# YifanXu74/MQ-Det

Hardware: AMD Instinct MI355X
Metric: images/sec MQ-GLIP-T 800×1333 5-shot vision queries, 1/2/4/8 MI355X (higher is better)
Workload: dtype f16; 1 GPU; BASELINE.json configs[1]: MQ-GLIP-T (Swin-T + BERT-base + GCP + 6-layer VLDyHead), 5 vision queries x 40 classes, 141-token caption, LVIS-style post-processing; every step a full forward (feature / language caches OFF; only host-side tokenizer / query-selection results are memoised)); global_batch=8, batch_per_gpu=8, image=800x1333 -> 800x1344, parallelism=dp1, weights=seeded random init (no checkpoints offline), residual_streams=fp32

## Files before the change

include/mqdet_hip.h:

```cpp
#ifndef MQDET_HIP_H
#define MQDET_HIP_H
#ifdef __cplusplus
extern "C" {
#endif

int mq_abi_version(void);

long mq_attn_workspace_bytes(int B, int H, int Nq, int D, int nsplit);
int mq_attn_fwd(const void* q, const void* k, const void* vt, void* o, const float* key_bias, const int* kv_len,
                const unsigned char* qk_mask, long mask_bs, long mask_hs, long mask_rs, void* workspace,
                int B, int H, int Nq, int Nk, int D,
                long q_bs, long q_rs, long q_hs, long k_bs, long k_rs, long k_hs, long vt_bs, long vt_rs, long vt_hs,
                long o_bs, long o_rs, long bias_bs, long bias_hs, float scale, float clamp, int nsplit, void* stream);

int mq_attn_resident_fwd(const void* q, const void* k, const void* vt, void* o, const float* key_bias, const int* kv_len,
                         const unsigned char* qk_mask, long mask_bs, long mask_hs, long mask_rs, int B, int H, int Nq, int Nk, int D,
                         long q_bs, long q_rs, long q_hs, long k_bs, long k_rs, long k_hs, long vt_bs, long vt_rs, long vt_hs,
                         long o_bs, long o_rs, long bias_bs, long bias_hs, float scale, float clamp, void* stream);

int mq_attn_chunked_fwd(const void* q, const void* k, const void* vt, void* o, const float* key_bias, const int* kv_len,
                        void* workspace, int B, int H, int Nq, int Nk, int D,
                        long q_bs, long q_rs, long q_hs, long k_bs, long k_rs, long k_hs, long vt_bs, long vt_rs, long vt_hs,
                        long o_bs, long o_rs, long bias_bs, long bias_hs, float scale, float clamp, int nsplit, void* stream);

// ... 80 lines not shown
int mq_add_upsample_nearest(void* dst, const void* src, int B, int H, int W, int Hc, int Wc, int C, void* stream);
int mq_dyrelu_ln_fwd(const void* x, long x_bs, const float* coef, const int* row_first, int NL, const void* gamma, const void* beta,
                     float eps, void* y, int B, int N, int C, void* stream);

int mq_align_scores_fwd(const void* dot, int dot_f32, const float* tbias, const int* tokidx, long tok_bs, const void* ctr,
                        float* out, float* cls_out, int B, int HW, int T, int L, int MT, float thr, long dot_bs, int agg,
                        void* stream);

int mq_align_fused_fwd(const void* tok, const void* tk, const float* tbias, const void* wbc, const float* bbc, const float* scales,
                       const int* tokidx, long tok_bs, const int* lvl_off, float* ranked, float* cls_out, float* reg, float* ctr_out,
                       float* logits, int B, int N, int T, int kv_max, int L, int MT, int NL, float thr, int agg, void* stream);

int mq_box_decode(const float* val, const long* flat, const void* reg, int reg_f32, const float* anchors, const int* label_ids, long lab_bs,
                  const float* im_wh, float* boxes, float* scores, int* labels, int B, int K, int HW, int L,
                  long out_stride, long out_off, void* stream);

int mq_roi_align_fwd(const void* feat, int feat_f32, const float* rois, float* out, int R, int C, int H, int W,
                     long sn, long sc, long sh, long sw, int PH, int PW, float spatial_scale, int sampling_ratio,
                     int aligned, int reduce_mean, void* stream);

int mq_msdeform_attn_fwd(const void* value, int value_f32, const long* shapes, const long* level_start, const float* loc,
                         const float* attn, void* out, int out_f32, int B, int S, int M, int D, int L, int Q, int P, void* stream);

int mq_msdeform_attn_q_fwd(const void* value, int value_f32, long value_bs, long value_ts, const long* shapes,
                           const long* level_start, const void* qproj, const float* ref, int ref_dim, const int* valid_hw,
                           void* out, int out_f32, int B, int S, int M, int D, int L, int Q, int P, void* stream);

long mq_ml_nms_workspace_bytes(int B, int N);
int mq_ml_nms(const float* boxes, const int* labels, const int* nvalid, void* workspace, unsigned char* keep,
              int B, int N, float thr, void* stream);

int mq_ml_nms_topk(const float* boxes, const int* labels, const int* nvalid, void* workspace, unsigned char* keep,
                   int B, int N, float thr, int max_keep, void* stream);

int mq_patch_embed_fwd(const void* img, int img_f32, const void* w, const float* bias, const float* g0, const float* b0, const float* g1,
                       const float* b1, float* x32, void* h1, int B, int Hi, int Wi, int C, float eps, void* stream);

int mq_attn_text_fwd(const void* q, const void* k, const void* v, void* o, const float* key_bias, const int* kv_len,
                     int B, int H, int Nq, int Nk, int D, long q_bs, long q_rs, long q_hs, long k_bs, long k_rs, long k_hs,
                     long v_bs, long v_rs, long v_hs, long o_bs, long o_rs, long bias_bs, long bias_hs, float scale,
                     float clamp, int max_kv, void* stream);

long mq_post_select_workspace_bytes(const int* hw, const int* k, int NL, int B, int L);
int mq_post_select_fwd(const float* const* ranked, const float* const* reg, const float* const* anchors, const int* hw, const int* k,
                       int NL, int B, int L, const int* label_ids, long lab_bs, const float* im_wh, void* workspace, float* boxes,
                       float* scores, int* labels, int* ids, void* stream);
int mq_post_sort_fwd(const float* boxes, const float* scores, const int* labels, const int* off, int NL, float* boxes_o, float* scores_o,
                     int* labels_o, int* nvalid, int B, int tot, void* stream);
int mq_post_finalize_fwd(const float* boxes, const float* scores, const int* labels, const unsigned char* keep, float* out,
                         int* counts, int B, int tot, int K, int K2, void* stream);

int mq_tta_ingest_fwd(const unsigned char* src, const long* src_off, const int* meta, const int* bounds, const int* coef, float* out,
                      float* out_flip, int* err, int B, int Hp, int Wp, int TH, int R, const float* mean, const float* stdv, int bgr, int x255,
                      void* stream);
int mq_tta_merge_prep(const float* packed, const int* counts, const float* tparam, const float* band, const int* cls_rank,
                      int n_cls, float* boxes, float* scores, int* labels, unsigned char* valid, float* boxes_s, float* scores_s,
                      int* labels_s, int* src_s, int* nvalid, int* ndrop, int T, int B, int K, void* stream);
int mq_tta_merge_finalize(const float* boxes_s, const float* scores_s, const int* labels_s, const int* src_s, const unsigned char* keep,
                          const int* nvalid, float* thr, const int* cls_rank, float* boxes_o, float* scores_o, long long* labels_o, int* counts, int B, int N,
                          int top_n, void* stream);
int mq_tta_merge_special(const float* boxes_s, const float* scores_s, const int* labels_s, const int* src_s, const int* nvalid,
                         const int* cls_rank, float* boxes_m, float* scores_m, unsigned char* keep, int* seq, float* ws, int* nws, int B,
                         int N, int L, int mode, float thresh, float aux, int cap, void* stream);
int mq_tta_merge_finalize_special(const float* boxes_m, const float* scores_m, const int* labels_s, const int* seq,
                                  const unsigned char* keep, const int* nvalid, float* thr, const int* cls_rank, float* boxes_o,
                                  float* scores_o, long long* labels_o, int* counts, int B, int N, int top_n, void* stream);
// ... 130 lines not shown
```

mq_det_amd/build.py:

```python
import os
import subprocess
import sys

HERE = os.path.dirname(os.path.abspath(__file__))
CSRC = os.path.join(HERE, "csrc")
LIB_DIR = os.path.join(HERE, "lib")
LIB = os.path.join(LIB_DIR, "libmqdet_hip.so")
SOURCES = ["api.hip", "attn.hip", "attn_resident.hip", "attn_text.hip", "bert_attn.hip", "vlfuse_attn.hip", "window_attn.hip", "patch_embed.hip", "gcp.hip", "gcp_fused.hip", "conv_igemm.hip", "conv_small.hip", "conv_small2.hip", "conv_small3.hip", "dcn_fused.hip", "layernorm.hip", "layernorm2.hip", "dyconv.hip", "post.hip", "post2.hip", "align_fused.hip", "nms2.hip", "roi_align.hip", "swin_mlp2.hip", "msda.hip", "tta.hip", "lvis_eval.hip", "coco_eval.hip", "flickr_eval.hip", "query_bank.hip"]
F32_SKIP = ("roi_align.hip", "nms2.hip", "post2.hip", "tta.hip", "lvis_eval.hip", "coco_eval.hip", "flickr_eval.hip", "query_bank.hip")
FLAGS = ["--offload-arch=gfx950", "-O3", "-std=c++17", "-fPIC"]
EXTRA_FLAGS = {"dcn_fused.hip": ["-fno-slp-vectorize"],
               "swin_mlp2.hip": ["-fno-slp-vectorize"],
               "attn_resident.hip": ["-fno-slp-vectorize", "-mllvm", "-amdgpu-mfma-vgpr-form"],
               "attn_text.hip": ["-fno-slp-vectorize", "-mllvm", "-amdgpu-mfma-vgpr-form"],
               "bert_attn.hip": ["-fno-slp-vectorize", "-mllvm", "-amdgpu-mfma-vgpr-form"]}


STAMP = os.path.join(LIB_DIR, "libmqdet_hip.stamp")


def _digest():
    import hashlib
    h = hashlib.sha256()
    deps = sorted(os.path.join(CSRC, f) for f in os.listdir(CSRC)) + [os.path.join(HERE, "..", "include", "mqdet_hip.h"), os.path.abspath(__file__)]
    for d in deps:
        if os.path.isfile(d):
            with open(d, "rb") as f:
                h.update(os.path.basename(d).encode() + b"\0" + f.read())
    return h.hexdigest()


def _stale():
    if not os.path.exists(LIB) or not os.path.exists(STAMP):
        return True
    with open(STAMP) as f:
        return f.read().strip() != _digest()


def build(force=False, verbose=True):
    if not force and not _stale():
        return LIB
    os.makedirs(LIB_DIR, exist_ok=True)
# ... 29 lines not shown
```

mq_det_amd/csrc/nms2.hip:

```cpp
#include "common.h"

MQ_NAMESPACE_BEGIN
#ifdef MQ_PRIMARY_UNIT

__device__ __forceinline__ float ml_iou2(const float* a, int la, const float* b, int lb) {
  if (la != lb) return 0.f;
  float left = fmaxf(a[0], b[0]), right = fminf(a[2], b[2]);
  float top = fmaxf(a[1], b[1]), bottom = fminf(a[3], b[3]);
  float w = fmaxf(right - left + 1.f, 0.f), h = fmaxf(bottom - top + 1.f, 0.f);
  float inter = w * h;
  float sa = (a[2] - a[0] + 1.f) * (a[3] - a[1] + 1.f);
  float sb = (b[2] - b[0] + 1.f) * (b[3] - b[1] + 1.f);
  return inter / (sa + sb - inter);
}

__global__ __launch_bounds__(64) void nms2_mask_kernel(const float* __restrict__ boxes, const int* __restrict__ labels,
                                                      const int* __restrict__ nvalid, unsigned long long* __restrict__ mask,
                                                      int N, int col_blocks, float thr) {
  const int b = blockIdx.z, row_blk = blockIdx.y, col_blk = blockIdx.x;
  const int n = nvalid[b];
  if (row_blk * 64 >= n || col_blk * 64 >= n || col_blk < row_blk) {
    int i = row_blk * 64 + threadIdx.x;
    if (i < N) mask[((long)b * N + i) * col_blocks + col_blk] = 0ULL;
    return;
  }
  __shared__ float cb[64 * 4];
  __shared__ int cl[64];
  const float* bb = boxes + (long)b * N * 4;
  const int* lb = labels + (long)b * N;
  const int cj = col_blk * 64 + threadIdx.x;
  if (cj < n) {
    cb[threadIdx.x * 4 + 0] = bb[cj * 4 + 0]; cb[threadIdx.x * 4 + 1] = bb[cj * 4 + 1];
    cb[threadIdx.x * 4 + 2] = bb[cj * 4 + 2]; cb[threadIdx.x * 4 + 3] = bb[cj * 4 + 3];
    cl[threadIdx.x] = lb[cj];
  }
  __syncthreads();
  const int i = row_blk * 64 + threadIdx.x;
  unsigned long long t = 0ULL;
  if (i < n) {
    float a[4] = {bb[i * 4 + 0], bb[i * 4 + 1], bb[i * 4 + 2], bb[i * 4 + 3]};
    int la = lb[i];
    int cols = min(64, n - col_blk * 64);
    int start = (row_blk == col_blk) ? threadIdx.x + 1 : 0;
    for (int j = start; j < cols; ++j)
      if (ml_iou2(a, la, cb + j * 4, cl[j]) > thr) t |= 1ULL << j;
  }
  if (i < N) mask[((long)b * N + i) * col_blocks + col_blk] = t;
// ... 116 lines not shown
```

mq_det_amd/ops.py:

```python
import ctypes
import math
import os

import torch

_LIB = None
_LIB_PATH = os.path.join(os.path.dirname(os.path.abspath(__file__)), "lib", "libmqdet_hip.so")

_vp, _i, _l, _f = ctypes.c_void_p, ctypes.c_int, ctypes.c_long, ctypes.c_float
EXPECTED_ABI = 31
_SIGNATURES = {
    "mq_abi_version": (_i, []),
    "mq_attn_workspace_bytes": (_l, [_i, _i, _i, _i, _i]),
    "mq_attn_fwd": (_i, [_vp, _vp, _vp, _vp, _vp, _vp, _vp, _l, _l, _l, _vp, _i, _i, _i, _i, _i] + [_l] * 13 + [_f, _f, _i, _vp]),
    "mq_attn_resident_fwd": (_i, [_vp, _vp, _vp, _vp, _vp, _vp, _vp, _l, _l, _l, _i, _i, _i, _i, _i] + [_l] * 13 + [_f, _f, _vp]),
    "mq_patch_embed_fwd": (_i, [_vp, _i, _vp, _vp, _vp, _vp, _vp, _vp, _vp, _vp, _i, _i, _i, _i, _f, _vp]),
    "mq_attn_text_fwd": (_i, [_vp, _vp, _vp, _vp, _vp, _vp, _i, _i, _i, _i, _i] + [_l] * 13 + [_f, _f, _i, _vp]),
    "mq_bert_attn_qkv_fwd": (_i, [_vp, _vp, _vp, _vp, _vp, _vp, _i, _i, _i, _i, _l, _l, _l, _l, _l, _f, _f, _vp]),
    "mq_attn_chunked_fwd": (_i, [_vp, _vp, _vp, _vp, _vp, _vp, _vp, _i, _i, _i, _i, _i] + [_l] * 13 + [_f, _f, _i, _vp]),
    "mq_window_attn_fwd": (_i, [_vp, _vp, _vp, _vp, _i, _i, _i, _i, _i, _i, _i, _vp]),
    "mq_window_attn_qkv_fwd": (_i, [_vp, _vp, _vp, _vp, _vp, _i, _i, _i, _i, _i, _i, _i, _vp]),
    "mq_gcp_sparse_attn_fwd": (_i, [_vp, _vp, _vp, _vp, _i, _i, _i, _i, _i, _i, _vp]),
    "mq_gcp_gate_residual_fwd": (_i, [_vp, _vp, _vp, _vp, _i, _vp, _vp, _l, _i, _i, _vp]),
    "mq_gcp_attn_fwd": (_i, [_vp] * 16 + [_l, _i, _i, _i, _i, _i, _i, _i, _f, _i, _vp]),
# ... 6 lines not shown
    "mq_clamp_gelu_clamp": (_i, [_vp, _vp, _l, _f, _vp]),
    "mq_patch_merge_ln_fwd": (_i, [_vp, _i, _vp, _vp, _vp, _i, _i, _i, _i, _f, _vp]),
    "mq_swin_mlp2_fwd": (_i, [_vp, _vp, _vp, _vp, _f, _vp, _vp, _vp, _vp, _vp, _vp, _vp, _f, _vp, _l, _i, _i, _vp]),
    "mq_conv3x3_fwd": (_i, [_vp, _vp, _vp, _vp, _i, _i, _i, _i, _l, _i, _i, _i, _vp]),
    "mq_conv3x3_nchw32_fwd": (_i, [_vp, _vp, _vp, _vp, _i, _i, _i, _i, _l, _i, _vp]),
    "mq_conv3x3_nchw32_v2_fwd": (_i, [_vp, _vp, _vp, _vp, _i, _i, _i, _i, _l, _i, _vp]),
    "mq_conv3x3_nchw32_group_fwd": (_i, [_vp, _i, _vp, _vp, _i, _i, _i, _vp]),
    "mq_dcnv2_stats_blocks": (_i, [_i, _i, _i]),
    "mq_dcnv2_fwd": (_i, [_vp, _vp, _vp, _vp, _vp, _vp, _vp, _vp, _i, _i, _i, _i, _l, _i, _i, _i, _i, _i, _i, _vp]),
    "mq_dcnv2_group_fwd": (_i, [_vp, _i, _vp]),
    "mq_dyconv_stats": (_i, [_vp, _vp, _vp, _vp, _i, _i, _i, _i, _vp]),
    "mq_dyconv_coef": (_i, [_vp, _vp, _vp, _vp, _vp, _vp, _i, _i, _i, _i, _i, _f, _i, _vp]),
    "mq_dyconv_coef_group": (_i, [_vp, _i, _vp, _vp, _i, _i, _i, _f, _vp]),
    "mq_dyconv_fuse": (_i, [_vp, _vp, _i, _i, _vp, _vp, _i, _i, _vp, _vp, _i, _i, _i, _vp, _l, _vp, _i, _i, _i, _i, _vp]),
    "mq_dyrelu_coef": (_i, [_vp, _vp, _vp, _vp, _vp, _vp, _i, _i, _i, _vp]),
    "mq_dyconv_epilogue_group": (_i, [_vp, _i, _vp, _vp, _vp, _vp, _i, _i, _vp]),
    "mq_add_upsample_nearest": (_i, [_vp, _vp, _i, _i, _i, _i, _i, _i, _vp]),
    "mq_pool2x2_tokens_fwd": (_i, [_vp, _i, _vp, _i, _i, _vp]),
    "mq_dyrelu_ln_fwd": (_i, [_vp, _l, _vp, _vp, _i, _vp, _vp, _f, _vp, _i, _i, _i, _vp]),
    "mq_dyrelu_apply": (_i, [_vp, _vp, _i, _i, _i, _l, _vp]),
    "mq_align_scores_fwd": (_i, [_vp, _i, _vp, _vp, _l, _vp, _vp, _vp, _i, _i, _i, _i, _i, _f, _l, _i, _vp]),
    "mq_align_fused_fwd": (_i, [_vp, _vp, _vp, _vp, _vp, _vp, _vp, _l, _vp, _vp, _vp, _vp, _vp, _vp, _i, _i, _i, _i, _i, _i, _i, _f, _i, _vp]),
    "mq_box_decode": (_i, [_vp, _vp, _vp, _i, _vp, _vp, _l, _vp, _vp, _vp, _vp, _i, _i, _i, _i, _l, _l, _vp]),
    "mq_roi_align_fwd": (_i, [_vp, _i, _vp, _vp, _i, _i, _i, _i, _l, _l, _l, _l, _i, _i, _f, _i, _i, _i, _vp]),
    "mq_msdeform_attn_fwd": (_i, [_vp, _i, _vp, _vp, _vp, _vp, _vp, _i, _i, _i, _i, _i, _i, _i, _i, _vp]),
    "mq_msdeform_attn_q_fwd": (_i, [_vp, _i, _l, _l, _vp, _vp, _vp, _vp, _i, _vp, _vp, _i, _i, _i, _i, _i, _i, _i, _i, _vp]),
    "mq_post_select_workspace_bytes": (_l, [_vp, _vp, _i, _i, _i]),
    "mq_post_select_fwd": (_i, [_vp, _vp, _vp, _vp, _vp, _i, _i, _i, _vp, _l, _vp, _vp, _vp, _vp, _vp, _vp, _vp]),
    "mq_post_sort_fwd": (_i, [_vp, _vp, _vp, _vp, _i, _vp, _vp, _vp, _vp, _i, _i, _vp]),
    "mq_post_finalize_fwd": (_i, [_vp, _vp, _vp, _vp, _vp, _vp, _i, _i, _i, _i, _vp]),
    "mq_ml_nms_workspace_bytes": (_l, [_i, _i]),
    "mq_ml_nms_topk": (_i, [_vp, _vp, _vp, _vp, _vp, _i, _i, _f, _i, _vp]),
    "mq_ml_nms": (_i, [_vp, _vp, _vp, _vp, _vp, _i, _i, _f, _vp]),
    "mq_tta_ingest_fwd": (_i, [_vp] * 8 + [_i] * 5 + [_vp, _vp, _i, _i, _vp]),
    "mq_tta_merge_prep": (_i, [_vp] * 5 + [_i] + [_vp] * 10 + [_i, _i, _i, _vp]),
    "mq_tta_merge_finalize": (_i, [_vp] * 12 + [_i, _i, _i, _vp]),
    "mq_tta_merge_special": (_i, [_vp] * 12 + [_i, _i, _i, _i, _f, _f, _i, _vp]),
    "mq_tta_merge_finalize_special": (_i, [_vp] * 12 + [_i, _i, _i, _vp]),
    "mq_tta_merge_nms": (_i, [_vp] * 7 + [_i, _i, _i, _f, _i, _vp]),
    "mq_lvis_match": (_i, [_vp] * 13 + [_i, _l, _vp]),
    "mq_lvis_accumulate": (_i, [_vp] * 7 + [_i, _vp]),
    "mq_coco_match": (_i, [_vp] * 12 + [_i, _l, _vp]),
    "mq_coco_accumulate": (_i, [_vp] * 9 + [_i, _vp]),
    "mq_flickr_recall": (_i, [_vp] * 7 + [_i, _i, _vp]),
    "mq_flickr_tally": (_i, [_vp] * 5 + [_i, _i, _i, _vp]),
    "mq_bank_admit": (_i, [_vp] * 8 + [_i] * 8 + [_f, _vp]),
}
BF16_TWINS = ("mq_attn_fwd", "mq_attn_resident_fwd", "mq_attn_text_fwd", "mq_bert_attn_qkv_fwd", "mq_patch_embed_fwd", "mq_attn_chunked_fwd", "mq_window_attn_fwd", "mq_window_attn_qkv_fwd", "mq_gcp_sparse_attn_fwd", "mq_gcp_gate_residual_fwd", "mq_gcp_attn_fwd", "mq_vlfuse_i2t_fwd", "mq_vlfuse_t2i_fwd",
              "mq_layernorm_fwd", "mq_layernorm2_fwd", "mq_layernorm_clamp_fwd", "mq_clamp_gelu_clamp", "mq_patch_merge_ln_fwd", "mq_swin_mlp2_fwd", "mq_conv3x3_fwd", "mq_conv3x3_nchw32_fwd", "mq_conv3x3_nchw32_v2_fwd", "mq_conv3x3_nchw32_group_fwd", "mq_dcnv2_fwd", "mq_dcnv2_group_fwd",
              "mq_dyconv_stats", "mq_dyconv_coef", "mq_dyconv_coef_group", "mq_dyconv_fuse", "mq_dyrelu_coef", "mq_dyconv_epilogue_group", "mq_dyrelu_apply", "mq_dyrelu_ln_fwd", "mq_add_upsample_nearest", "mq_pool2x2_tokens_fwd",
              "mq_align_scores_fwd", "mq_align_fused_fwd", "mq_box_decode", "mq_roi_align_fwd", "mq_msdeform_attn_fwd", "mq_msdeform_attn_q_fwd")
F32_TWINS = tuple(n for n in BF16_TWINS if n not in ("mq_roi_align_fwd",))
for _n in BF16_TWINS:
    _SIGNATURES[_n + "_bf16"] = _SIGNATURES[_n]
for _n in F32_TWINS:
    _SIGNATURES[_n + "_f32"] = _SIGNATURES[_n]
EXPORTS = tuple(_SIGNATURES)


from .selection import KERNEL_DEFAULTS, KERNELS, _ThreadLocalTable, configure, activate


def lib_path():
    return _LIB_PATH


# ... 1196 lines not shown

def ms_deform_attn_q(value, spatial_shapes, qproj, ref, heads, out_dtype=None, valid_hw=None):
    lib = load_library()
    _need_gpu(value, qproj, ref)
    B, S, C = value.shape
    D = C // heads
    Q = qproj.shape[1]
    shapes = tuple((int(h), int(w)) for h, w in spatial_shapes)
    L, P = len(shapes), 4
    assert sum(h * w for h, w in shapes) == S and value.stride(2) == 1 and value.dtype in _H16 + (torch.float32,)
    assert qproj.dtype in _H16 and qproj.is_contiguous() and qproj.shape == (B, Q, heads * L * P * 3)
    assert ref.dtype == torch.float32 and ref.is_contiguous() and ref.shape[:3] == (B, Q, L) and ref.shape[3] in (2, 4)
    if valid_hw is not None:
        _need_gpu(valid_hw)
        assert valid_hw.dtype == torch.int32 and valid_hw.is_contiguous() and valid_hw.shape == (B, L, 2)
    hw, start = _msda_shapes(shapes, value.device)
    out_dtype = out_dtype or value.dtype
    out = torch.empty(B, Q, C, dtype=out_dtype, device=value.device)
    nb = B * S * C * value.element_size() + qproj.numel() * 2 + ref.numel() * 4 + out.numel() * out.element_size()
    with _timed(f"msdeform_attn_q{Q}", nb):
        _chk(_fn(lib, "mq_msdeform_attn_q_fwd", value, qproj, out)(_ptr(value), int(value.dtype == torch.float32), value.stride(0), value.stride(1), _ptr(hw),
                                        _ptr(start), _ptr(qproj), _ptr(ref), ref.shape[3], _ptr(valid_hw), _ptr(out),
                                        int(out_dtype == torch.float32), B, S, heads, D, L, Q, P, _stream()),
             "mq_msdeform_attn_q_fwd")
    return out


def ml_nms(boxes, labels, nvalid, thresh, max_keep=0, as_bool=True):
    lib = load_library()
    _need_gpu(boxes, labels, nvalid)
    B, N, _ = boxes.shape
    assert boxes.is_contiguous() and labels.is_contiguous() and boxes.dtype == torch.float32
    assert labels.dtype == torch.int32 and nvalid.dtype == torch.int32
    ws = torch.empty(max(lib.mq_ml_nms_workspace_bytes(B, N), 8), dtype=torch.uint8, device=boxes.device)
    keep = torch.empty(B, N, dtype=torch.uint8, device=boxes.device)
    if max_keep > 0 and N <= 6656 and KERNELS["NMS_EARLY_STOP"] == 1:
        _chk(lib.mq_ml_nms_topk(_ptr(boxes), _ptr(labels), _ptr(nvalid), _ptr(ws), _ptr(keep), B, N, float(thresh), int(max_keep), _stream()),
             "mq_ml_nms_topk")
        return keep.bool() if as_bool else keep
    _chk(lib.mq_ml_nms(_ptr(boxes), _ptr(labels), _ptr(nvalid), _ptr(ws), _ptr(keep), B, N, float(thresh), _stream()),
         "mq_ml_nms")
    return keep.bool() if as_bool else keep


TTA_MERGE_MAX_ROWS = 256 * 64
def tta_ingest(src, src_off, meta, bounds, coef, B, Hp, Wp, TH, R, mean, std, bgr, x255, flip, err):
    lib = load_library()
    _need_gpu(src, src_off, meta, bounds, coef, err)
    assert src.dtype == torch.uint8 and src_off.dtype == torch.int64 and meta.dtype == bounds.dtype == coef.dtype == torch.int32
    out = torch.empty(B, 3, Hp, Wp, dtype=torch.float32, device=src.device)
    out_f = torch.empty_like(out) if flip else None
    m, s = (ctypes.c_float * 3)(*[float(v) for v in mean]), (ctypes.c_float * 3)(*[float(v) for v in std])
    with _timed("tta_ingest", src.numel() + out.numel() * 4 * (2 if flip else 1)):
        _chk(lib.mq_tta_ingest_fwd(_ptr(src), _ptr(src_off), _ptr(meta), _ptr(bounds), _ptr(coef), _ptr(out), _ptr(out_f), _ptr(err), B, Hp, Wp, TH, R,
                                   ctypes.cast(m, ctypes.c_void_p), ctypes.cast(s, ctypes.c_void_p), int(bgr), int(x255), _stream()),
             "mq_tta_ingest_fwd")
    return out, out_f


TTA_SPECIAL_MODES = {"none": 0, "soft-nms": 1, "vote": 2, "soft-vote": 3}
TTA_SOFT_NMS_SIGMA = 0.95
TTA_SPECIAL_ROW_CAP = 1024
TTA_SPECIAL_MAX_CAP = 4096
TTA_NMS_ROW_CAP = 4096
TTA_MERGE_MAX_ROWS_ANY = 1 << 24
TTA_NMS_PATHS = ("auto", "segmented")
# ... 215 lines not shown
```

mq_det_amd/selection.py:

```python
import os

KERNEL_DEFAULTS = {
    "LN_VARIANT": 2,
    "OFFSET_CONV_VARIANT": 3,
    "PATCH_MERGE_FUSED": 1,
    "FPN_VIA_DCN": 1,
    "NMS_EARLY_STOP": 1,
    "ATTN_RESIDENT": 1,
    "SWIN_MLP_VARIANT": 2,
    "SWIN_MLP2_FLAGS": -1,
    "SWIN_QKV_FUSED": 2,
    "FPN_TOPDOWN_FUSED": 1,
    "DYRELU_IN_LN": 1,
    "VLFUSE_I2T_VARIANT": 0,
    "SWIN_MLP_TAIL_STREAM": 0,
    "DYCONV_EPILOGUE_GROUPED": 1,
    "BERT_CLAMP_FUSED": 1,
    "PATCH_EMBED_FUSED": 1,
    "BERT_QKV_FUSED": 1,
    "FRONT_SIDE_STREAM": 1,
    "LANG_SIDE_STREAMS": 0,
    "GCP_ATTN_FUSED": 1,
    "BERT_ATTN_QKV_FUSED": 1,
    "POST_FUSED": 1,
    "F32_OPERANDS": 0,
    "DCN_BDMA": 1,
    "POOLED_TOKENS_FUSED": 1,
    "ALIGN_FUSED": 1,
}
class _ThreadLocalTable(dict):

    def __init__(self, init):
        super().__init__()
        import threading
        object.__setattr__(self, "_tl", threading.local())
        object.__setattr__(self, "_base", dict(init))

    def _cur(self):
        t = self._tl
        if not hasattr(t, "d"):
# ... 59 lines not shown
```

Measured before the change: 512.6 images/sec.

## Add class-partitioned multi-label NMS with per-class tiled suppression and early stop

```diff
diff --git a/include/mqdet_hip.h b/include/mqdet_hip.h
--- a/include/mqdet_hip.h
+++ b/include/mqdet_hip.h
@@ -136,6 +136,10 @@
 
 int mq_ml_nms_topk(const float* boxes, const int* labels, const int* nvalid, void* workspace, unsigned char* keep,
                    int B, int N, float thr, int max_keep, void* stream);
+
+long mq_ml_nms_classwise_workspace_bytes(int B, int N);
+int mq_ml_nms_classwise(const float* boxes, const int* labels, const int* nvalid, void* workspace, unsigned char* keep,
+                        int B, int N, float thr, int max_keep, void* stream);
 
 int mq_patch_embed_fwd(const void* img, int img_f32, const void* w, const float* bias, const float* g0, const float* b0, const float* g1,
                        const float* b1, float* x32, void* h1, int B, int Hi, int Wi, int C, float eps, void* stream);
diff --git a/mq_det_amd/build.py b/mq_det_amd/build.py
--- a/mq_det_amd/build.py
+++ b/mq_det_amd/build.py
@@ -6,8 +6,8 @@
 CSRC = os.path.join(HERE, "csrc")
 LIB_DIR = os.path.join(HERE, "lib")
 LIB = os.path.join(LIB_DIR, "libmqdet_hip.so")
-SOURCES = ["api.hip", "attn.hip", "attn_resident.hip", "attn_text.hip", "bert_attn.hip", "vlfuse_attn.hip", "window_attn.hip", "patch_embed.hip", "gcp.hip", "gcp_fused.hip", "conv_igemm.hip", "conv_small.hip", "conv_small2.hip", "conv_small3.hip", "dcn_fused.hip", "layernorm.hip", "layernorm2.hip", "dyconv.hip", "post.hip", "post2.hip", "align_fused.hip", "nms2.hip", "roi_align.hip", "swin_mlp2.hip", "msda.hip", "tta.hip", "lvis_eval.hip", "coco_eval.hip", "flickr_eval.hip", "query_bank.hip"]
-F32_SKIP = ("roi_align.hip", "nms2.hip", "post2.hip", "tta.hip", "lvis_eval.hip", "coco_eval.hip", "flickr_eval.hip", "query_bank.hip")
+SOURCES = ["api.hip", "attn.hip", "attn_resident.hip", "attn_text.hip", "bert_attn.hip", "vlfuse_attn.hip", "window_attn.hip", "patch_embed.hip", "gcp.hip", "gcp_fused.hip", "conv_igemm.hip", "conv_small.hip", "conv_small2.hip", "conv_small3.hip", "dcn_fused.hip", "layernorm.hip", "layernorm2.hip", "dyconv.hip", "post.hip", "post2.hip", "align_fused.hip", "nms2.hip", "nms3.hip", "roi_align.hip", "swin_mlp2.hip", "msda.hip", "tta.hip", "lvis_eval.hip", "coco_eval.hip", "flickr_eval.hip", "query_bank.hip"]
+F32_SKIP = ("roi_align.hip", "nms2.hip", "nms3.hip", "post2.hip", "tta.hip", "lvis_eval.hip", "coco_eval.hip", "flickr_eval.hip", "query_bank.hip")
 FLAGS = ["--offload-arch=gfx950", "-O3", "-std=c++17", "-fPIC"]
 EXTRA_FLAGS = {"dcn_fused.hip": ["-fno-slp-vectorize"],
                "swin_mlp2.hip": ["-fno-slp-vectorize"],
diff --git a/mq_det_amd/csrc/nms2.hip b/mq_det_amd/csrc/nms2.hip
--- a/mq_det_amd/csrc/nms2.hip
+++ b/mq_det_amd/csrc/nms2.hip
@@ -3,16 +3,7 @@
 MQ_NAMESPACE_BEGIN
 #ifdef MQ_PRIMARY_UNIT
 
-__device__ __forceinline__ float ml_iou2(const float* a, int la, const float* b, int lb) {
-  if (la != lb) return 0.f;
-  float left = fmaxf(a[0], b[0]), right = fminf(a[2], b[2]);
-  float top = fmaxf(a[1], b[1]), bottom = fminf(a[3], b[3]);
-  float w = fmaxf(right - left + 1.f, 0.f), h = fmaxf(bottom - top + 1.f, 0.f);
-  float inter = w * h;
-  float sa = (a[2] - a[0] + 1.f) * (a[3] - a[1] + 1.f);
-  float sb = (b[2] - b[0] + 1.f) * (b[3] - b[1] + 1.f);
-  return inter / (sa + sb - inter);
-}
+#include "nms_iou.h"
 
 __global__ __launch_bounds__(64) void nms2_mask_kernel(const float* __restrict__ boxes, const int* __restrict__ labels,
                                                       const int* __restrict__ nvalid, unsigned long long* __restrict__ mask,
diff --git a/mq_det_amd/csrc/nms3.hip b/mq_det_amd/csrc/nms3.hip
--- /dev/null
+++ b/mq_det_amd/csrc/nms3.hip
@@ -0,0 +1,551 @@
+#include "common.h"
+
+MQ_NAMESPACE_BEGIN
+#ifdef MQ_PRIMARY_UNIT
+#include "nms_iou.h"
+
+#define NMS3_MED 256
+#define NMS3_MAXLONG 32
+#define NMS3_WAVES 4
+
+struct Nms3Ws {
+  int* order;
+  float* sbox;
+  int* mseg;
+  int* hdr;
+  int* ltab;
+  unsigned long long* tiles;
+};
+static inline __host__ __device__ long nms3_off_sbox(int N) { return (long)((N + 3) & ~3) * 4; }
+static inline __host__ __device__ long nms3_off_mseg(int N) { return nms3_off_sbox(N) + (long)N * 16; }
+static inline __host__ __device__ long nms3_off_hdr(int N) { return nms3_off_mseg(N) + (long)((N / 2 + 2) & ~1) * 8; }
+static inline __host__ __device__ long nms3_off_ltab(int N) { return nms3_off_hdr(N) + 16; }
+static inline __host__ __device__ long nms3_off_tiles(int N) { return nms3_off_ltab(N) + NMS3_MAXLONG * 16; }
+static inline __host__ __device__ long nms3_image_bytes(int N) {
+  const long cb = (N + 63) / 64;
+  return nms3_off_tiles(N) + cb * (cb + 1) / 2 * 512;
+}
+__device__ __forceinline__ Nms3Ws nms3_ws(unsigned char* ws, int b, int N) {
+  unsigned char* w = ws + (long)b * nms3_image_bytes(N);
+  Nms3Ws r;
+  r.order = (int*)w;
+  r.sbox = (float*)(w + nms3_off_sbox(N));
+  r.mseg = (int*)(w + nms3_off_mseg(N));
+  r.hdr = (int*)(w + nms3_off_hdr(N));
+  r.ltab = (int*)(w + nms3_off_ltab(N));
+  r.tiles = (unsigned long long*)(w + nms3_off_tiles(N));
+  return r;
+}
+__device__ __forceinline__ int nms3_block_off(int nch, int c) { return 64 * (c * nch - c * (c - 1) / 2); }
+
+__device__ __forceinline__ unsigned long long nms3_peers(int d, int valid) {
+  unsigned long long peers = __ballot(valid);
+#pragma unroll
+  for (int bit = 0; bit < 8; ++bit) {
+    const int on = (d >> bit) & 1;
+    const unsigned long long m = __ballot(valid && on);
+    peers &= on ? m : ~m;
+  }
+  return peers;
+}
+
+__global__ __launch_bounds__(1024) void nms3_partition_kernel(const float* __restrict__ boxes, const int* __restrict__ labels,
+                                                             const int* __restrict__ nvalid, unsigned char* __restrict__ ws,
+                                                             unsigned char* __restrict__ keep, int N, int P) {
+  extern __shared__ __attribute__((aligned(16))) unsigned key_s[];
+  __shared__ int cnt_s[256 * 16];
+  __shared__ int wsum_s[16];
+  __shared__ int nlong_s;
+  __shared__ int long_s[NMS3_MAXLONG * 2];
+  unsigned short* row_s = (unsigned short*)(key_s + 2 * (P + 4));
+  const int b = blockIdx.x, tid = threadIdx.x, lane = tid & 63, wave = tid >> 6;
+  const int n = min(max(nvalid[b], 0), N);
+  const float* bb = boxes + (long)b * N * 4;
+  const int* lb = labels + (long)b * N;
+  unsigned char* kb = keep + (long)b * N;
+  const Nms3Ws w = nms3_ws(ws, b, N);
+  for (int i = tid; i < n; i += 1024) { key_s[i] = (unsigned)lb[i]; row_s[i] = (unsigned short)i; }
+  if (tid == 0) nlong_s = 0;
+  {
+    unsigned x = 0u;
+    const unsigned l0 = n > 0 ? (unsigned)lb[0] : 0u;
+    for (int i = tid; i < n; i += 1024) x |= (unsigned)lb[i] ^ l0;
+#pragma unroll
+    for (int o = 32; o > 0; o >>= 1) x |= __shfl_xor(x, o);
+    if (lane == 0) wsum_s[wave] = (int)x;
+  }
+  __syncthreads();
+  unsigned diffbits = 0u;
+  for (int x = 0; x < 16; ++x) diffbits |= (unsigned)wsum_s[x];
+  const int R = 64 * ((n + 1023) / 1024);
+  const unsigned long long lt_mask = (1ULL << lane) - 1ULL;
+  int cur = 0;
+  for (int pass = 0; pass < 4; ++pass) {
+    const int shift = 8 * pass;
+    if (((diffbits >> shift) & 255u) == 0u) continue;
+    const unsigned* kin = key_s + cur * (P + 4);
+    const unsigned short* rin = row_s + cur * P;
+    unsigned* kout = key_s + (cur ^ 1) * (P + 4);
+    unsigned short* rout = row_s + (cur ^ 1) * P;
+    for (int i = tid; i < 256 * 16; i += 1024) cnt_s[i] = 0;
+    __syncthreads();
+    for (int q = 0; q < R; q += 64) {
+      const int p = wave * R + q + lane, valid = p < n;
+      const int d = valid ? (int)((kin[p] >> shift) & 255) : 0;
+      const unsigned long long peers = nms3_peers(d, valid);
+      if (valid) {
+        if ((peers & lt_mask) == 0ULL) cnt_s[d * 16 + wave] += __popcll(peers);
+      }
+      wave_lds_fence();
+    }
+    __syncthreads();
+    {
+      const int a0 = cnt_s[4 * tid], a1 = cnt_s[4 * tid + 1], a2 = cnt_s[4 * tid + 2], a3 = cnt_s[4 * tid + 3];
+      int v = a0 + a1 + a2 + a3;
+      for (int d = 1; d < 64; d <<= 1) {
+        const int t = __shfl(v, max(lane - d, 0));
+        if (lane >= d) v += t;
+      }
+      if (lane == 63) wsum_s[wave] = v;
+      __syncthreads();
+      int base = v - (a0 + a1 + a2 + a3);
+      for (int x = 0; x < wave; ++x) base += wsum_s[x];
+      cnt_s[4 * tid] = base;
+      cnt_s[4 * tid + 1] = base + a0;
+      cnt_s[4 * tid + 2] = base + a0 + a1;
+      cnt_s[4 * tid + 3] = base + a0 + a1 + a2;
+    }
+    __syncthreads();
+    for (int q = 0; q < R; q += 64) {
+      const int p = wave * R + q + lane, valid = p < n;
+      const unsigned key = valid ? kin[p] : 0u;
+      const int d = (int)((key >> shift) & 255);
+      const unsigned long long peers = nms3_peers(d, valid);
+      if (valid) {
+        const int dst = cnt_s[d * 16 + wave] + __popcll(peers & lt_mask);
+        kout[dst] = key;
+        rout[dst] = rin[p];
+      }
+      wave_lds_fence();
+      if (valid && (peers & lt_mask) == 0ULL) cnt_s[d * 16 + wave] += __popcll(peers);
+      wave_lds_fence();
+    }
+    __syncthreads();
+    cur ^= 1;
+  }
+  __syncthreads();
+  const unsigned* kfin = key_s + cur * (P + 4);
+  const unsigned short* rfin = row_s + cur * P;
+  int* seg_s = (int*)(key_s + (cur ^ 1) * (P + 4));
+#pragma unroll 2
+  for (int p = tid; p < n; p += 1024) {
+    const int row = (int)rfin[p];
+    const float x0 = bb[row * 4 + 0], x1 = bb[row * 4 + 1], x2 = bb[row * 4 + 2], x3 = bb[row * 4 + 3];
+    w.order[p] = row;
+    kb[row] = 0;
+    w.sbox[p * 4 + 0] = x0;
+    w.sbox[p * 4 + 1] = x1;
+    w.sbox[p * 4 + 2] = x2;
+    w.sbox[p * 4 + 3] = x3;
+  }
+  const int IT = (n + 1023) / 1024, base = tid * IT;
+  auto label_at = [&](int p) { return kfin[p]; };
+  auto flags_at = [&](int p) {
+    const unsigned l = label_at(p);
+    const int head = p == 0 || label_at(p - 1) != l;
+    const int multi = head && p + 1 < n && label_at(p + 1) == l;
+    return head | (multi << 16);
+  };
+  int loc = 0;
+  for (int q = 0; q < IT; ++q)
+    if (base + q < n) loc += flags_at(base + q);
+  int v = loc;
+  for (int d = 1; d < 64; d <<= 1) {
+    const int t = __shfl(v, max(lane - d, 0));
+    if (lane >= d) v += t;
+  }
+  if (lane == 63) wsum_s[wave] = v;
+  __syncthreads();
+  int excl = v - loc, total = 0;
+  for (int x = 0; x < 16; ++x) {
+    if (x < wave) excl += wsum_s[x];
+    total += wsum_s[x];
+  }
+  const int nseg = total & 0xffff, nmulti = total >> 16;
+  {
+    int sid = excl & 0xffff;
+    for (int q = 0; q < IT; ++q) {
+      const int p = base + q;
+      if (p >= n) break;
+      const int f = flags_at(p), row = (int)rfin[p];
+      if (f & 1) {
+        seg_s[sid++] = p;
+        if (!(f >> 16)) kb[row] = 1;
+      }
+    }
+    if (tid == 0) seg_s[nseg] = n;
+  }
+  __syncthreads();
+  {
+    int sid = excl & 0xffff, mid = excl >> 16;
+    for (int q = 0; q < IT; ++q) {
+      const int p = base + q;
+      if (p >= n) break;
+      const int f = flags_at(p);
+      if (f >> 16) {
+        const int end = seg_s[sid + 1];
+        w.mseg[2 * mid] = p;
+        w.mseg[2 * mid + 1] = end;
+        ++mid;
+        if (end - p > NMS3_MED) {
+          const int k = atomicAdd(&nlong_s, 1);
+          long_s[2 * k] = p;
+          long_s[2 * k + 1] = end;
+        }
+      }
+      if (f & 1) ++sid;
+    }
+  }
+  __syncthreads();
+  if (tid == 0) {
+    const int nl = nlong_s;
+    for (int i = 1; i < nl; ++i) {
+      const int s = long_s[2 * i], e = long_s[2 * i + 1];
+      int j = i - 1;
+      for (; j >= 0 && (long_s[2 * j + 1] - long_s[2 * j] > e - s || (long_s[2 * j + 1] - long_s[2 * j] == e - s && long_s[2 * j] > s)); --j) { long_s[2 * j + 2] = long_s[2 * j]; long_s[2 * j + 3] = long_s[2 * j + 1]; }
+      long_s[2 * j + 2] = s;
+      long_s[2 * j + 3] = e;
+    }
+    int tile0 = 0;
+    for (int k = 0; k < nl; ++k) {
+      const int s = long_s[2 * k], e = long_s[2 * k + 1], nch = (e - s + 63) / 64;
+      w.ltab[4 * k + 0] = s;
+      w.ltab[4 * k + 1] = e;
+      w.ltab[4 * k + 2] = tile0;
+      w.ltab[4 * k + 3] = nch;
+      tile0 += nch * (nch + 1) / 2;
+    }
+    w.hdr[0] = nmulti;
+    w.hdr[1] = nl;
+    w.hdr[2] = tile0;
+    w.hdr[3] = 0;
+  }
+}
+
+__device__ __forceinline__ unsigned long long nms3_uniform(unsigned long long v) {
+  return ((unsigned long long)(unsigned)__builtin_amdgcn_readfirstlane((int)(v >> 32)) << 32) | (unsigned)__builtin_amdgcn_readfirstlane((int)v);
+}
+#if defined(MQ_SIMT_EMULATION)
+#define NMS3_READLANE(v, j) __shfl((v), (j))
+#else
+#define NMS3_READLANE(v, j) __builtin_amdgcn_readlane((v), (j))
+#endif
+__device__ __forceinline__ unsigned long long nms3_chain(unsigned long long m, unsigned long long diag) {
+  const int lo = (int)diag, hi = (int)(diag >> 32);
+#pragma unroll
+  for (int j = 0; j < 64; ++j) {
+    const unsigned long long dj = ((unsigned long long)(unsigned)NMS3_READLANE(hi, j) << 32) | (unsigned)NMS3_READLANE(lo, j);
+    m &= ((m >> j) & 1ULL) ? ~dj : ~0ULL;
+  }
+  return m;
+}
+__device__ __forceinline__ unsigned long long nms3_tile(const float* __restrict__ sbox, int s, int e, int c, int cc, float* cb, int lane, float thr) {
+  wave_lds_fence();
+  const int pc = s + cc * 64 + lane;
+  if (pc < e) {
+    cb[lane * 4 + 0] = sbox[pc * 4 + 0]; cb[lane * 4 + 1] = sbox[pc * 4 + 1];
+    cb[lane * 4 + 2] = sbox[pc * 4 + 2]; cb[lane * 4 + 3] = sbox[pc * 4 + 3];
+  }
+  wave_lds_fence();
+  const int pr = s + c * 64 + lane;
+  unsigned long long bits = 0ULL;
+  if (pr < e) {
+    const float a[4] = {sbox[pr * 4 + 0], sbox[pr * 4 + 1], sbox[pr * 4 + 2], sbox[pr * 4 + 3]};
+    const int cols = min(64, e - (s + cc * 64));
+#pragma unroll 4
+    for (int j = 0; j < cols; ++j)
+      if (ml_iou2(a, 0, cb + j * 4, 0) > thr) bits |= 1ULL << j;
+    if (c == cc) bits &= ~((2ULL << lane) - 1ULL);
+  }
+  return bits;
+}
+__device__ __forceinline__ void nms3_tile_index(int nch, int u, int& c, int& cc) {
+  c = 0;
+  while (u >= nch - c) { u -= nch - c; ++c; }
+  cc = c + u;
+}
+
+__global__ __launch_bounds__(64 * NMS3_WAVES) void nms3_resolve_kernel(unsigned char* __restrict__ ws, unsigned char* __restrict__ keep,
+                                                                      int N, float thr) {
+  __shared__ __attribute__((aligned(16))) float cb_s[NMS3_WAVES][64 * 4];
+  __shared__ unsigned long long bits_s[NMS3_MED / 64 * (NMS3_MED / 64 + 1) / 2][64];
+  const int b = blockIdx.y, wave = threadIdx.x >> 6, lane = threadIdx.x & 63;
+  const int wid = blockIdx.x * NMS3_WAVES + wave, nwaves = gridDim.x * NMS3_WAVES;
+  const Nms3Ws w = nms3_ws(ws, b, N);
+  unsigned char* kb = keep + (long)b * N;
+  float* cb = cb_s[wave];
+  const int nmulti = w.hdr[0], nlong = w.hdr[1], ntiles = w.hdr[2];
+
+  for (int m = wid; m < nmulti; m += nwaves) {
+    const int s = w.mseg[2 * m], e = w.mseg[2 * m + 1];
+    if (e - s > 64) continue;
+    const int row = s + lane < e ? w.order[s + lane] : 0;
+    const unsigned long long alive = nms3_chain(__ballot(s + lane < e), nms3_tile(w.sbox, s, e, 0, 0, cb, lane, thr));
+    if (s + lane < e) kb[row] = (unsigned char)((alive >> lane) & 1ULL);
+  }
+
+  for (int m = blockIdx.x; m < nmulti; m += gridDim.x) {
+    const int s = w.mseg[2 * m], e = w.mseg[2 * m + 1];
+    if (e - s <= 64 || e - s > NMS3_MED) continue;
+    const int nch = (e - s + 63) / 64, T = nch * (nch + 1) / 2;
+    for (int u = wave; u < T; u += NMS3_WAVES) {
+      int c, cc;
+      nms3_tile_index(nch, u, c, cc);
+      bits_s[u][lane] = nms3_tile(w.sbox, s, e, c, cc, cb, lane, thr);
+    }
+    __syncthreads();
+    if (wave == 0) {
+      unsigned long long remv[NMS3_MED / 64];
+#pragma unroll
+      for (int c = 0; c < NMS3_MED / 64; ++c) remv[c] = 0ULL;
+#pragma unroll
+      for (int c = 0; c < NMS3_MED / 64; ++c) {
+        if (c < nch) {
+          const int p = s + c * 64 + lane, t0 = c * nch - c * (c - 1) / 2;
+          const int row = p < e ? w.order[p] : 0;
+          const unsigned long long alive = nms3_chain(__ballot(p < e) & ~remv[c], bits_s[t0][lane]);
+          if (p < e) kb[row] = (unsigned char)((alive >> lane) & 1ULL);
+#pragma unroll
+          for (int cc = c + 1; cc < NMS3_MED / 64; ++cc) {
+            if (cc < nch) {
+              unsigned long long acc = ((alive >> lane) & 1ULL) ? bits_s[t0 + cc - c][lane] : 0ULL;
+#pragma unroll
+              for (int o = 32; o > 0; o >>= 1) acc |= __shfl_xor(acc, o);
+              remv[cc] |= nms3_uniform(acc);
+            }
+          }
+        }
+      }
+    }
+    __syncthreads();
+  }
+
+  int k = 0;
+  for (int t = wid; t < ntiles; t += nwaves) {
+    while (k + 1 < nlong && t >= w.ltab[4 * (k + 1) + 2]) ++k;
+    const int s = w.ltab[4 * k], e = w.ltab[4 * k + 1], tile0 = w.ltab[4 * k + 2];
+    const int nch = (e - s + 63) / 64;
+    int c, cc;
+    nms3_tile_index(nch, t - tile0, c, cc);
+    const unsigned long long bits = nms3_tile(w.sbox, s, e, c, cc, cb, lane, thr);
+    w.tiles[(long)tile0 * 64 + nms3_block_off(nch, c) + lane * (nch - c) + (cc - c)] = bits;
+  }
+}
+
+template <int SLOTS>
+__global__ __launch_bounds__(1024) void nms3_sweep_kernel(unsigned char* __restrict__ ws, const int* __restrict__ nvalid, unsigned char* keep,
+                                                        int N, int max_keep) {
+  extern __shared__ __attribute__((aligned(16))) unsigned long long rows_s[];
+  __shared__ int ctl_s[2];
+  __shared__ int zr_s[NMS3_MAXLONG * 2];
+  __shared__ int nz_s;
+  __shared__ int cnt_s[128];
+  __shared__ int cend_s;
+  __shared__ int lt_s[NMS3_MAXLONG * 4];
+  __shared__ int ord_s[3][65];
+  typedef unsigned long long u64x2 __attribute__((ext_vector_type(2)));
+  const int b = blockIdx.x, tid = threadIdx.x, wave = tid >> 6, lane = tid & 63;
+  const int n = min(max(nvalid[b], 0), N);
+  const Nms3Ws w = nms3_ws(ws, b, N);
+  unsigned char* kb = keep + (long)b * N;
+  const int bufw = 64 * ((N + 63) / 64);
+  const int nlong = w.hdr[1];
+  if (tid < 4 * nlong) lt_s[tid] = w.ltab[tid];
+  __syncthreads();
+  auto nch_of = [&](int k) { return (lt_s[4 * k + 1] - lt_s[4 * k] + 63) / 64; };
+  auto advance = [&](int& k, int& c) {
+    if (k >= nlong) return;
+    if (++c >= nch_of(k)) { ++k; c = 0; }
+  };
+  constexpr int U = 11, NL = 320;
+  const int grp = wave > 0 ? (wave - 1) / 5 : 0, lt = tid - 64 - grp * NL;
+  u64x2 pv[U];
+  int pord = 0, pslot = -1, pwords = 0;
+  auto issue = [&](int k, int c, int slot) {
+    pslot = -1;
+    if (k >= nlong) return;
+    const int nch = nch_of(k);
+    const unsigned long long* src = w.tiles + (long)lt_s[4 * k + 2] * 64 + nms3_block_off(nch, c);
+    pwords = 64 * (nch - c);
+    pslot = slot;
+#pragma unroll
+    for (int u = 0; u < U; ++u) {
+      const int idx = (u * NL + lt) * 2;
+      pv[u] = (u64x2){0ULL, 0ULL};
+      if (idx < pwords) pv[u] = *(const u64x2*)(src + idx);
+    }
+    if (lt < 65) {
+      const int pp = lt_s[4 * k] + c * 64 + lt;
+      pord = pp < lt_s[4 * k + 1] ? w.order[pp] : 0;
+    }
+  };
+  auto commit = [&]() {
+    if (pslot < 0) return;
+    unsigned long long* dst = rows_s + pslot * bufw;
+#pragma unroll
+    for (int u = 0; u < U; ++u) {
+      const int idx = (u * NL + lt) * 2;
+      if (idx < pwords) *(u64x2*)(dst + idx) = pv[u];
+    }
+    if (lt < 65) ord_s[pslot][lt] = pord;
+    pslot = -1;
+  };
+  int k = 0, c = 0, q = 0;
+  auto prime = [&]() {
+    int kk = k, cc = c;
+    for (int j = 0; j < 3; ++j) {
+      if (grp == (q + j) % 3) {
+        issue(kk, cc, (q + j) % 3);
+        if (j == 0) {
+          commit();
+          int k3 = kk, c3 = cc;
+          for (int a = 0; a < 3; ++a) advance(k3, c3);
+          issue(k3, c3, q % 3);
+        }
+      }
+      advance(kk, cc);
+    }
+  };
+  if (wave > 0) prime();
+  if (tid < 2) ctl_s[tid] = 0;
+  if (tid == 0) nz_s = 0;
+  const int nchk = (n + 63) / 64;
+  for (int ch = wave; ch < nchk; ch += 16) {
+    const int i = ch * 64 + lane;
+    const unsigned long long m = __ballot(i < n && kb[i] != 0);
+    if (lane == 0) cnt_s[ch] = __popcll(m);
+  }
+  __syncthreads();
+  int reached = 0, c_reach = 0, acc_lt = 0, c_acc = 0;
+  unsigned long long remv[SLOTS];
+  while (k < nlong) {
+    int k1 = k, c1 = c;
+    advance(k1, c1);
+    if (wave > 0) {
+      if (grp == (q + 1) % 3) {
+        int k4 = k1, c4 = c1;
+        for (int a = 0; a < 3; ++a) advance(k4, c4);
+        commit();
+        issue(k4, c4, (q + 1) % 3);
+      }
+    } else {
+      const int s = lt_s[4 * k], e = lt_s[4 * k + 1], nch = (e - s + 63) / 64, pitch = nch - c;
+      const unsigned long long* L = rows_s + (q % 3) * bufw;
+      if (c == 0) {
+        reached = 0; c_reach = 0; acc_lt = 0; c_acc = 0;
+#pragma unroll
+        for (int sl = 0; sl < SLOTS; ++sl) remv[sl] = 0ULL;
+      }
+      const int p0 = s + c * 64, p = p0 + lane, have = p < e, pn0 = p0 + 64;
+      const int row = ord_s[q % 3][lane];
+      const int rown0 = ord_s[q % 3][64];
+      unsigned long long word = 0ULL;
+#pragma unroll
+      for (int sl = 0; sl < SLOTS; ++sl)
+        if (sl == c / 64) word = remv[sl];
+      word = __shfl(word, c % 64);
+      const unsigned long long alive_mask = nms3_chain(__ballot(have && !((word >> lane) & 1ULL)), have ? L[lane * pitch] : 0ULL);
+      const int alive = (int)((alive_mask >> lane) & 1ULL);
+      if (have) kb[row] = (unsigned char)alive;
+      if (alive) atomicAdd(&cnt_s[row >> 6], 1);
+      wave_lds_fence();
+      if (!reached) {
+        c_reach = __builtin_amdgcn_readfirstlane(__shfl(row, min(63, e - p0 - 1)) >> 6);
+        for (; c_acc < c_reach; ++c_acc) acc_lt += cnt_s[c_acc];
+        reached = acc_lt + cnt_s[c_reach] >= max_keep;
+      }
+      const int end_seg = reached && pn0 < e && rown0 / 64 > c_reach;
+      if (end_seg) {
+        if (lane == 0) {
+          ctl_s[q & 1] = q + 1;
+          zr_s[2 * nz_s] = pn0;
+          zr_s[2 * nz_s + 1] = e;
+          nz_s = nz_s + 1;
+        }
+      } else if (pn0 < e) {
+        for (int r0 = 0; r0 < 64; r0 += 8) {
+          if (((alive_mask >> r0) & 0xFFULL) == 0ULL) continue;
+          unsigned long long v[8][SLOTS];
+#pragma unroll
+          for (int kk = 0; kk < 8; ++kk)
+#pragma unroll
+            for (int sl = 0; sl < SLOTS; ++sl) {
+              const int cc = lane + 64 * sl;
+              v[kk][sl] = (cc > c && cc < nch) ? L[(r0 + kk) * pitch + (cc - c)] : 0ULL;
+            }
+#pragma unroll
+          for (int kk = 0; kk < 8; ++kk)
+            if ((alive_mask >> (r0 + kk)) & 1ULL) {
+#pragma unroll
+              for (int sl = 0; sl < SLOTS; ++sl) remv[sl] |= v[kk][sl];
+            }
+        }
+      }
+    }
+    __syncthreads();
+    if (ctl_s[q & 1] == q + 1) {
+      ++k; c = 0; ++q;
+      if (k >= nlong) break;
+      if (wave > 0) prime();
+      __syncthreads();
+      continue;
+    }
+    k = k1; c = c1; ++q;
+  }
+  __syncthreads();
+  const int nz = nz_s;
+  for (int z = 0; z < nz; ++z)
+    for (int p = zr_s[2 * z] + tid; p < zr_s[2 * z + 1]; p += 1024) kb[w.order[p]] = 0;
+  __syncthreads();
+  if (wave == 0) {
+    int v0 = lane < nchk ? cnt_s[lane] : 0, v1 = lane + 64 < nchk ? cnt_s[lane + 64] : 0;
+    for (int d = 1; d < 64; d <<= 1) {
+      const int t0 = __shfl(v0, max(lane - d, 0)), t1 = __shfl(v1, max(lane - d, 0));
+      if (lane >= d) { v0 += t0; v1 += t1; }
+    }
+    v1 += __shfl(v0, 63);
+    const unsigned long long m0 = __ballot(lane < nchk && v0 >= max_keep), m1 = __ballot(lane + 64 < nchk && v1 >= max_keep);
+    if (lane == 0) cend_s = m0 ? __ffsll(m0) : m1 ? 64 + __ffsll(m1) : nchk;
+  }
+  __syncthreads();
+  const int lim = min(cend_s * 64, n);
+  for (int i = lim + tid; i < N; i += 1024) kb[i] = 0;
+}
+
+extern "C" long mq_ml_nms_classwise_workspace_bytes(int B, int N) {
+  if (B <= 0 || N <= 0) return 0;
+  return (long)B * nms3_image_bytes(N);
+}
+
+extern "C" int mq_ml_nms_classwise(const float* boxes, const int* labels, const int* nvalid, void* workspace, unsigned char* keep,
+                                   int B, int N, float thr, int max_keep, void* stream) {
+  if (B <= 0 || N <= 0) return 0;
+  if (max_keep < 1) return -2;
+  const int col_blocks = (N + 63) / 64;
+  if (col_blocks > 104) return -1;
+  const int P = (N + 63) & ~63;
+  const size_t smem1 = (size_t)2 * (P + 4) * 4 + (size_t)2 * P * 2;
+  int rc = mq_launch<nms3_partition_kernel>(dim3(B), dim3(1024), smem1, (hipStream_t)stream, boxes, labels, nvalid, (unsigned char*)workspace, keep,
+                                            N, P);
+  if (rc) return rc;
+  const int groups = min(1024, max(4, (col_blocks * (col_blocks + 1) / 2 + NMS3_WAVES - 1) / NMS3_WAVES));
+  hipLaunchKernelGGL(nms3_resolve_kernel, dim3(groups, B), dim3(64 * NMS3_WAVES), 0, (hipStream_t)stream, (unsigned char*)workspace, keep, N, thr);
+  MQ_CHECK_LAUNCH();
+  const size_t smem3 = (size_t)3 * 64 * col_blocks * sizeof(unsigned long long);
+  if (col_blocks <= 64)
+    return mq_launch<nms3_sweep_kernel<1>>(dim3(B), dim3(1024), smem3, (hipStream_t)stream, (unsigned char*)workspace, nvalid, keep, N, max_keep);
+  return mq_launch<nms3_sweep_kernel<2>>(dim3(B), dim3(1024), smem3, (hipStream_t)stream, (unsigned char*)workspace, nvalid, keep, N, max_keep);
+}
+#endif
+
+MQ_NAMESPACE_END
diff --git a/mq_det_amd/csrc/nms_iou.h b/mq_det_amd/csrc/nms_iou.h
--- /dev/null
+++ b/mq_det_amd/csrc/nms_iou.h
@@ -0,0 +1,13 @@
+#pragma once
+
+__device__ __forceinline__ float ml_iou2(const float* a, int la, const float* b, int lb) {
+#pragma clang fp contract(off)
+  if (la != lb) return 0.f;
+  float left = fmaxf(a[0], b[0]), right = fminf(a[2], b[2]);
+  float top = fmaxf(a[1], b[1]), bottom = fminf(a[3], b[3]);
+  float w = fmaxf(right - left + 1.f, 0.f), h = fmaxf(bottom - top + 1.f, 0.f);
+  float inter = w * h;
+  float sa = (a[2] - a[0] + 1.f) * (a[3] - a[1] + 1.f);
+  float sb = (b[2] - b[0] + 1.f) * (b[3] - b[1] + 1.f);
+  return inter / (sa + sb - inter);
+}
diff --git a/mq_det_amd/ops.py b/mq_det_amd/ops.py
--- a/mq_det_amd/ops.py
+++ b/mq_det_amd/ops.py
@@ -62,6 +62,8 @@
     "mq_ml_nms_workspace_bytes": (_l, [_i, _i]),
     "mq_ml_nms_topk": (_i, [_vp, _vp, _vp, _vp, _vp, _i, _i, _f, _i, _vp]),
     "mq_ml_nms": (_i, [_vp, _vp, _vp, _vp, _vp, _i, _i, _f, _vp]),
+    "mq_ml_nms_classwise_workspace_bytes": (_l, [_i, _i]),
+    "mq_ml_nms_classwise": (_i, [_vp, _vp, _vp, _vp, _vp, _i, _i, _f, _i, _vp]),
     "mq_tta_ingest_fwd": (_i, [_vp] * 8 + [_i] * 5 + [_vp, _vp, _i, _i, _vp]),
     "mq_tta_merge_prep": (_i, [_vp] * 5 + [_i] + [_vp] * 10 + [_i, _i, _i, _vp]),
     "mq_tta_merge_finalize": (_i, [_vp] * 12 + [_i, _i, _i, _vp]),
@@ -1324,6 +1326,12 @@
     B, N, _ = boxes.shape
     assert boxes.is_contiguous() and labels.is_contiguous() and boxes.dtype == torch.float32
     assert labels.dtype == torch.int32 and nvalid.dtype == torch.int32
+    if max_keep > 0 and N <= 6656 and KERNELS["NMS_EARLY_STOP"] == 1 and KERNELS["NMS_CLASSWISE"] == 1:
+        ws = torch.empty(max(lib.mq_ml_nms_classwise_workspace_bytes(B, N), 8), dtype=torch.uint8, device=boxes.device)
+        keep = torch.empty(B, N, dtype=torch.uint8, device=boxes.device)
+        _chk(lib.mq_ml_nms_classwise(_ptr(boxes), _ptr(labels), _ptr(nvalid), _ptr(ws), _ptr(keep), B, N, float(thresh), int(max_keep), _stream()),
+             "mq_ml_nms_classwise")
+        return keep.bool() if as_bool else keep
     ws = torch.empty(max(lib.mq_ml_nms_workspace_bytes(B, N), 8), dtype=torch.uint8, device=boxes.device)
     keep = torch.empty(B, N, dtype=torch.uint8, device=boxes.device)
     if max_keep > 0 and N <= 6656 and KERNELS["NMS_EARLY_STOP"] == 1:
diff --git a/mq_det_amd/selection.py b/mq_det_amd/selection.py
--- a/mq_det_amd/selection.py
+++ b/mq_det_amd/selection.py
@@ -6,6 +6,7 @@
     "PATCH_MERGE_FUSED": 1,
     "FPN_VIA_DCN": 1,
     "NMS_EARLY_STOP": 1,
+    "NMS_CLASSWISE": 1,
     "ATTN_RESIDENT": 1,
     "SWIN_MLP_VARIANT": 2,
     "SWIN_MLP2_FLAGS": -1,
```

New measurement: 501.2 images/sec. 2.2% lower.
